# Symb0x76/ChineseChessZero

Measured on AMD Instinct MI355X. Metric: self-play MCTS simulations/sec, higher is better.
Workload: dtype u8 rules / f32 Q (reference CPU path) / f64 PUCT (net: fp16)

## Files before the change

chinesechesszero_amd/_lib.py:

```python
from __future__ import annotations

import ctypes as C
import os

import torch

_HERE = os.path.dirname(os.path.abspath(__file__))
LIB_PATH = os.path.join(_HERE, "libcczero.so")

NSQ = 90
SQ_STRIDE = 96
NMOVES = 2086
MAX_LEGAL = 128
MASK_WORDS = 66
PLANES = 10710
REC_BYTES, REC_HDR, REC_IDS, REC_PI = 880, 96, 112, 368
HEAD_POL_STRIDE, HEAD_VAL_STRIDE = 1536, 640

ABI_VERSION = 8
CONV_RELU, CONV_DESCENDING, CONV_FORCE_SMALL, CONV_FORCE_TILE, CONV_G16, CONV_G16_EDGE_TILES = 1, 2, 16, 32, 64, 128
CONV_G16_ONE_LAUNCH = 512
RULE_PERPETUAL_CHECK = 1
RULE_PAWN_MOVE_RESETS_CLOCK = 2
FLAG_REFERENCE_QUIRKS = 1
# ... 46 lines not shown
    "ccz_last_error": (C.c_char_p, []),
    "ccz_device_count": (C.c_int, []),
    "ccz_action_table": (C.c_int, [_P, _P, _P]),
    "ccz_flip_map": (C.c_int, [_P]),
    "ccz_create": (C.c_int, [C.POINTER(Config), C.POINTER(_P)]),
    "ccz_destroy": (C.c_int, [_P]),
    "ccz_reset": (C.c_int, [_P, _P, _P]),
    "ccz_set_position": (C.c_int, [_P, _P, C.c_int32, _P, C.c_int32, C.c_int32]),
    "ccz_reset_tree": (C.c_int, [_P, _P, _P]),
    "ccz_select_leaves": (C.c_int, [_P, _P, _P]),
    "ccz_zero_leaf_input": (C.c_int, [_P, _P, _P]),
    "ccz_expand_backup": (C.c_int, [_P, _P, _P, _P]),
    "ccz_step": (C.c_int, [_P, _P, _P, _P, _P]),
    "ccz_gather_priors": (C.c_int, [_P, _P, _P, C.c_int32]),
    "ccz_step_compact": (C.c_int, [_P, _P, _P, _P]),
    "ccz_expand_backup_compact": (C.c_int, [_P, _P, _P]),
    "ccz_eval_plan": (C.c_int, [_P, _P, _P, _P]),
    "ccz_set_scouts": (C.c_int, [_P, C.c_int32]),
    "ccz_scout": (C.c_int, [_P, _P, _P]),
    "ccz_eval_plan_scouted": (C.c_int, [_P, _P, _P, _P, _P]),
    "ccz_scout_and_plan": (C.c_int, [_P, _P, _P, _P, _P, _P]),
    "ccz_scouted_run": (C.c_int, [_P, _P, _P, _P, _P, _P, _P]),
    "ccz_gather_priors_planned": (C.c_int, [_P, _P, _P, C.c_int32, _P]),
    "ccz_eval_cache_clear": (C.c_int, [_P, _P]),
    "ccz_set_routing": (C.c_int, [_P, _P, _P, C.c_uint64, C.c_uint64]),
    "ccz_eval_plan_routed": (C.c_int, [_P, _P, _P, _P]),
    "ccz_gather_priors_routed": (C.c_int, [_P, _P, _P, _P, C.c_int32, _P, _P]),
    "ccz_finish_move": (C.c_int, [_P, _P, _P, _P, _P, C.c_int32]),
    "ccz_root_children": (C.c_int, [_P, _P, _P, _P, _P, _P, _P, _P]),
    "ccz_root_pi": (C.c_int, [_P, _P, _P, _P]),
    "ccz_move_distribution": (C.c_int, [_P, _P, _P, _P, _P, _P]),
    "ccz_game_status": (C.c_int, [_P, _P, _P, _P, _P, _P]),
    "ccz_root_positions": (C.c_int, [_P, _P, _P]),
    "ccz_leaf_info": (C.c_int, [_P, _P, _P, _P, _P, _P]),
    "ccz_leaf_priors": (C.c_int, [_P, _P, _P, _P]),
    "ccz_leaf_keys": (C.c_int, [_P, _P, _P, _P]),
    "ccz_harvest_rows": (C.c_int, [_P, _P, C.POINTER(C.c_int64)]),
    "ccz_harvest": (C.c_int, [_P, _P, _P, _P, _P, C.c_int64, C.POINTER(C.c_int64)]),
    "ccz_harvest_records": (C.c_int, [_P, _P, _P, C.c_int64, C.POINTER(C.c_int64)]),
    "ccz_expand_records": (C.c_int, [_P, _P, C.c_int64, C.c_uint32, _P, _P, _P, _P, C.c_int64, C.c_int64, _P]),
    "ccz_ring_retire": (C.c_int, [_P, _P, C.c_int64, _P, C.c_int64, C.c_int32, _P]),
    "ccz_sample_records": (C.c_int, [_P, _P, C.c_int64, _P, _P, C.c_int64, C.c_uint32, _P, _P, _P, _P, _P]),
    "ccz_get_stats": (C.c_int, [_P, _P, C.POINTER(Stats)]),
    "ccz_legal_moves": (C.c_int, [_P, C.c_int32, _P, _P, _P, _P, _P, _P]),
    "ccz_apply_moves": (C.c_int, [_P, C.c_int32, _P, _P, _P, _P]),
    "ccz_bias_act_f16": (C.c_int, [_P, _P, _P, _P, C.c_int64, C.c_int32]),
# ... 73 lines not shown
```

chinesechesszero_amd/csrc/cczero.hip:

```cpp
#include "../../include/cczero.h"

#include <hip/hip_runtime.h>

#include <cmath>
#include <cstdarg>
#include <cstdio>
#include <cstring>
#include <new>
#include <vector>

#include "cczero_kernels.h"
#include "cczero_netops.h"
#include "cczero_conv.h"
#include "cczero_conv_small.h"
#include "cczero_conv_g16.h"
#include "cczero_conv_g16e.h"
#include "cczero_heads.h"

using namespace ccz;

namespace {

thread_local char g_err[512] = "";

// ... 504 lines not shown
    return 0;
}

int ccz_eval_cache_clear(ccz_engine *e, void *stream)
{
    NEED(e);
    if (!e->d.cache) return 0;
    hipStream_t s = (hipStream_t)stream;
    HIP_TRY(hipMemsetAsync(e->d.cache, 0, ((size_t)e->d.cache_mask + 1) * sizeof(CacheEntry), s));
    HIP_TRY(hipMemsetAsync(e->d.claim, 0x7f, ((size_t)e->d.cache_mask + 1) * 4, s));
    return 0;
}

int ccz_step_compact(ccz_engine *e, void *stream, const float *value_dev, void *leaf_input_f16_dev)
{
    NEED(e);
    if (!value_dev && !e->d.cache) return fail(-1, "ccz_step_compact: null value (engine-owned leaf values exist only with an evaluation cache)");
    hipLaunchKernelGGL(k_step<true>, dim3(ACTIVE(e)), dim3(64), 0, (hipStream_t)stream, e->d, (const float *)e->d.prior128, value_dev,
                       (uint16_t *)leaf_input_f16_dev);
    HIP_TRY(hipGetLastError());
    return 0;
}

int ccz_expand_backup_compact(ccz_engine *e, void *stream, const float *value_dev)
{
    NEED(e);
    if (!value_dev && !e->d.cache) return fail(-1, "ccz_expand_backup_compact: null value (engine-owned leaf values exist only with an evaluation cache)");
    hipLaunchKernelGGL(k_expand_backup<true>, dim3(ACTIVE(e)), dim3(64), 0, (hipStream_t)stream, e->d, (const float *)e->d.prior128,
                       value_dev);
    HIP_TRY(hipGetLastError());
    return 0;
}

int ccz_finish_move(ccz_engine *e, void *stream, const int32_t *forced_moves_dev, const double *temps_dev,
                    int32_t *moves_out_dev, int32_t keep_tree)
{
    NEED(e);
    hipLaunchKernelGGL(k_finish_move, dim3(ACTIVE(e)), dim3(64), 0, (hipStream_t)stream, e->d, forced_moves_dev, temps_dev,
                       moves_out_dev, keep_tree ? 1 : 0);
    HIP_TRY(hipGetLastError());
    hipLaunchKernelGGL(k_flip_half, dim3(1), dim3(1), 0, (hipStream_t)stream, e->d);
    HIP_TRY(hipGetLastError());
    return 0;
}

int ccz_root_children(ccz_engine *e, void *stream, int32_t *k_host, uint16_t *acts_host, int32_t *visits_host,
// ... 663 lines not shown
```

chinesechesszero_amd/csrc/cczero_kernels.h:

```cpp
#pragma once
#include "cczero_device.h"

namespace ccz {

constexpr uint16_t kHalfOne = 0x3C00;
constexpr int kMaxDepth = 512;

__device__ __forceinline__ void set_err(const Dev &D, int bit) { atomicOr(D.err, bit); }

__device__ __forceinline__ int start_piece(int s)
{
    const int r = s / 9, f = s - 9 * r;
    const int rr = r <= 4 ? r : 9 - r;
    const int add = r <= 4 ? 0 : 8;
    int t = 0;
    if (rr == 0) {
        const int ff = f <= 4 ? f : 8 - f;
        t = ff == 0 ? ROOK : ff == 1 ? KNIGHT : ff == 2 ? BISHOP : ff == 3 ? ADVISOR : KING;
    } else if (rr == 2) {
        t = (f == 1 || f == 7) ? CANNON : 0;
    } else if (rr == 3) {
        t = (f & 1) ? 0 : PAWN;
    }
    return t ? t + add : 0;
// ... 399 lines not shown
        if (lane == 0) { D.leaf_status[b] = CCZ_LEAF_NONE; D.leaf_k[b] = 0; D.path_len[b] = 0; }
        return;
    }
    if (lane < 24) {
        uint32_t v = P.sqw;
        if (lane == 22) v &= 0x0000ffffu;
        if (lane == 23) v = 0u;
        ((uint32_t *)sh.sq)[lane] = v;
    }
    sh.chain[lane] = P.c0;
    if (P.m.chain_len > 64) sh.chain[64 + lane] = D.chain[(size_t)r * kChainCap + 64 + lane];
    if (lane >= 1 && lane < d) sh.pm.mv[lane - 1] = (uint16_t)(Bn[CCZ_IDX(D, pj, D.cap)] & 0xffffu);
    if (lane == 0) sh.pm.mv[d - 1] = (uint16_t)(Bn[CCZ_IDX(D, sib, D.cap)] & 0xffffu);
    wave_sync();
    leaf_tail(D, b, lane, leaf_in, sh, d, P.m.turn, P.m.halfmove, P.m.chain_len, P.m.key, false);
}

__global__ __launch_bounds__(64) void k_scout(Dev D, uint16_t *leaf_in, int active)
{
    __shared__ SelectShared sh;
    scout_wave(D, leaf_in, active, blockIdx.x, threadIdx.x, sh);
}

template <bool COMPACT>
__device__ inline TopPatch expand_backup_phase(const Dev &D, int b, int lane, const float *prob, const float *value,
                                               const BoardMeta &m0, int half)
{
    TopPatch tp;
    tp.active = false; tp.root_expanded = false; tp.kid_expanded = false; tp.k = 0; tp.first_id = 0; tp.n0 = 0; tp.rootN = 0;
    tp.rootQ = 0.0f; tp.node1 = -1; tp.N1 = 0; tp.Q1 = 0.0f; tp.has1 = false;
    const int status = D.leaf_status[b];
    const int d = D.path_len[b];
    const int k_leaf = D.leaf_k[b];
    const float v_net = value ? value[b] : D.vleaf[b];
    const int32_t *path = D.path + (size_t)b * D.maxd;
    const uint16_t *ids = D.leaf_ids + (size_t)b * kMaxLegal;
    const int id0 = ids[lane], id1 = ids[64 + lane];
    float cp0 = 0.0f, cp1 = 0.0f;
    if (COMPACT) { cp0 = prob[(size_t)b * kMaxLegal + lane]; cp1 = prob[(size_t)b * kMaxLegal + 64 + lane]; }
    const int pj = path[lane < D.maxd ? lane : 0];
    if (status == CCZ_LEAF_SKIP) return tp;
    CCZ_STAMP(D, b, lane, 8)
    BoardMeta *mp = D.meta + b;
    const size_t base = ((size_t)b * 2 + half) * (size_t)D.cap;
    NodeA *A = D.nodeA + base;
    uint32_t *Bn = D.nodeB + base;
    const int leaf = __builtin_amdgcn_readlane(pj, __builtin_amdgcn_readfirstlane(d < 64 ? d : 0));
    float v;
    if (status == CCZ_LEAF_EXPAND) {
        const int k = k_leaf;
        const int n0 = m0.n_nodes;
        v = v_net;
        if (n0 + k > D.cap) {
            set_err(D, 1);
        } else {
            const float *pr = prob + (size_t)b * kNMoves;
            if (lane < k) {
                A[CCZ_IDX(D, n0 + lane, D.cap)] = NodeA{0, 0.0f, COMPACT ? cp0 : pr[COMPACT ? 0 : CCZ_IDX(D, id0, kNMoves)], -1};
                Bn[CCZ_IDX(D, n0 + lane, D.cap)] = (uint32_t)id0;
            }
            if (64 + lane < k) {
                A[CCZ_IDX(D, n0 + 64 + lane, D.cap)] = NodeA{0, 0.0f, COMPACT ? cp1 : pr[COMPACT ? 0 : CCZ_IDX(D, id1, kNMoves)], -1};
// ... 69 lines not shown
    __shared__ SelectShared sh;
    const int b = blockIdx.x, lane = threadIdx.x;
    CCZ_STAMP(D, b, lane, 0)
    const Prefetch P = prefetch_board(D, b, lane);
    const TopPatch tp = expand_backup_phase<COMPACT>(D, b, lane, prob, value, P.m, P.half);
    CCZ_STAMP(D, b, lane, 1)
    __threadfence_block();
    __syncthreads();
    CCZ_STAMP(D, b, lane, 2)
    select_phase(D, b, lane, leaf_in, sh, P, tp);
    CCZ_STAMP(D, b, lane, 9)
}

__device__ __forceinline__ uint32_t cache_tag(int id0, int id1, int k, int lane)
{
    uint64_t h = 0;
    if (lane < k) h ^= mix64(((uint64_t)(uint32_t)id0 << 8 | (uint32_t)lane) + 0x9E3779B97F4A7C15ull);
    if (64 + lane < k) h ^= mix64(((uint64_t)(uint32_t)id1 << 8 | (uint32_t)(64 + lane)) + 0x9E3779B97F4A7C15ull);
    h = wave_readlane64(wave_incl_xor64(h), 63);
    return ((uint32_t)(h >> 40) << 8) | (uint32_t)(k & 0xff);
}

template <typename T, bool PLANNED>
__device__ __forceinline__ void softmax_gather_board(const Dev &D, int b, int lane, float *row, const T *logits, const float *vcompact,
                                                     uint64_t salt)
{
    const int status = D.leaf_status[b];
    int cst = 0, src = b;
    if (PLANNED) {
        cst = D.cstate[b];
        src = D.row_of[b];
    }
    const int k = D.leaf_k[b];
    const uint16_t *ids = D.leaf_ids + (size_t)b * kMaxLegal;
    const int id0 = ids[lane], id1 = ids[64 + lane];
    if (status != CCZ_LEAF_EXPAND || cst != 0) return;
    const T *srcrow = logits + (size_t)src * kNMoves;
    float mx = -__builtin_huge_valf();
    float sum = 0.0f;
    if constexpr (sizeof(T) == 2) {
        static_assert(kNMoves % 2 == 0, "dword rows");
        const uint32_t *src32 = (const uint32_t *)srcrow;
        constexpr int kIt = (kNMoves / 2 + 63) / 64;
        uint32_t wreg[kIt];
#pragma unroll
        for (int i = 0; i < kIt; ++i) {
            const int j = lane + 64 * i;
            wreg[i] = j < kNMoves / 2 ? src32[j] : 0u;
        }
#pragma unroll
        for (int i = 0; i < kIt; ++i) {
            const int j = lane + 64 * i;
            if (j < kNMoves / 2) {
                const uint32_t w = wreg[i];
                const float x0 = (float)__builtin_bit_cast(_Float16, (uint16_t)(w & 0xffffu));
                const float x1 = (float)__builtin_bit_cast(_Float16, (uint16_t)(w >> 16));
                *(float2 *)(row + 2 * j) = make_float2(x0, x1);
                mx = fmaxf(mx, fmaxf(x0, x1));
            }
// ... 24 lines not shown
            const bool d0 = lane < k && __float_as_uint(out[lane]) != __float_as_uint(p0);
            const bool d1 = 64 + lane < k && __float_as_uint(out[64 + lane]) != __float_as_uint(p1);
            const bool dv = __float_as_uint(D.vleaf[b]) != __float_as_uint(v);
            const bool bad = __ballot(d0 || d1 || dv) != 0ull;
            if (lane == 0) {
                D.stats[b].cache_verified += 1u;
                if (bad) D.stats[b].cache_mismatch += 1u;
            }
        }
        if (lane < k) out[lane] = p0;
        if (64 + lane < k) out[64 + lane] = p1;
        const uint32_t slot = D.cslot[b];
        if (lane == 0) {
            D.vleaf[b] = v;
            D.claim[slot] = 0x7fffffff;
        }
        if (D.cins[b]) {
            CacheEntry *e = D.cache + slot;
            const uint32_t tag = cache_tag(id0, id1, k, lane);
            e->pri[lane] = p0;
            e->pri[64 + lane] = p1;
            if (lane == 0) { e->v = v; e->k = tag; e->key = D.leaf_key[b] ^ salt; D.stats[b].cache_stores += 1u; }
        }
    } else {
        if (lane < k) out[lane] = p0;
        if (64 + lane < k) out[64 + lane] = p1;
    }
}

template <typename T, bool PLANNED>
__global__ __launch_bounds__(64) void k_softmax_gather(Dev D, const T *logits, const float *vcompact)
{
    __shared__ __attribute__((aligned(16))) float row[kNMoves + 2];
    softmax_gather_board<T, PLANNED>(D, blockIdx.x, threadIdx.x, row, logits, vcompact, 0ull);
}

template <typename T>
__global__ __launch_bounds__(64) void k_softmax_gather_routed(Dev D, const uint8_t *net, const T *logits0, const T *logits1,
                                                              const float *v0, const float *v1, uint64_t salt0, uint64_t salt1)
{
    __shared__ __attribute__((aligned(16))) float row[kNMoves + 2];
    const int b = blockIdx.x;
    const int n = net[b];
    softmax_gather_board<T, true>(D, b, threadIdx.x, row, n ? logits1 : logits0, n ? v1 : v0, n ? salt1 : salt0);
}

__device__ __forceinline__ uint32_t cache_slot(uint64_t key, uint32_t mask) { return (uint32_t)(key ^ (key >> 29)) & mask; }

__device__ inline int cache_probe_wave(const Dev &D, int b, int lane, uint64_t salt = 0)
{
    const int status = D.leaf_status[b];
    const uint64_t key = D.leaf_key[b] ^ salt;
    if (status != CCZ_LEAF_EXPAND) {
        if (lane == 0) D.cstate[b] = 2;
        return 2;
    }
    const uint32_t slot = cache_slot(key, D.cache_mask);
// ... 887 lines not shown
```

chinesechesszero_amd/engine.py:

```python
from __future__ import annotations

import ctypes as C

import numpy as np
import torch

from . import _lib
from ._lib import MAX_LEGAL, NMOVES, SQ_STRIDE, CczError, Config, Stats, check


def _ptr(t):
    if t is None:
        return None
    if isinstance(t, torch.Tensor):
        return C.c_void_p(t.data_ptr())
    if isinstance(t, np.ndarray):
        return C.c_void_p(t.ctypes.data)
    raise TypeError(type(t))


class SelfPlayEngine:
    def __init__(self, n_boards: int, n_playout: int = 400, c_puct: float = 5, eps: float = 0.25,
                 alpha: float = 0.2, temp: float = 1.0, seed: int = 0, board_id_base: int = 0,
                 device: int = 0, max_nodes: int = 0, max_depth: int = 0, max_plies: int = 0,
# ... 31 lines not shown
            cfg.move_rank_host = self.move_rank.ctypes.data
        self.plane_of_type = (0, 0, 1, 2, 3, 4, 5, 6) if plane_of_type is None else tuple(int(x) for x in plane_of_type)
        if plane_of_type is not None:
            cfg.plane_of_type = (C.c_uint8 * 8)(*self.plane_of_type)
        if isinstance(pawn_move_resets_clock, str):
            pawn_move_resets_clock = tools.PAWN_MOVE_RESETS_CLOCK
        self.pawn_move_resets_clock = bool(pawn_move_resets_clock)
        if isinstance(perpetual_check, str):
            perpetual_check = tools.PERPETUAL_CHECK
        self.perpetual_check = bool(perpetual_check)
        cfg.rule_flags = (_lib.RULE_PAWN_MOVE_RESETS_CLOCK if self.pawn_move_resets_clock else 0) \
            | (_lib.RULE_PERPETUAL_CHECK if self.perpetual_check else 0)
        self.type_rank = None if type_rank is None else tuple(int(x) for x in type_rank)
        if self.type_rank is not None:
            if len(self.type_rank) != 8:
                raise ValueError("type_rank must have 8 entries")
            cfg.type_rank = (C.c_uint8 * 8)(*self.type_rank)
        self.eval_cache_log2 = int(eval_cache_log2)
        cfg.eval_cache_log2 = self.eval_cache_log2
        h = C.c_void_p()
        with torch.cuda.device(self.device):
            check(self.L.ccz_create(C.byref(cfg), C.byref(h)))
        self.h = h
        self.miss_rows = torch.zeros((self.B,), dtype=torch.int32, device=self.device)
        self.n_miss = torch.zeros((1,), dtype=torch.int32, device=self.device)
        self.leaf_input = torch.zeros((self.B, 17, 7, 10, 9), dtype=torch.float16, device=self.device)
        self.moves_out = torch.full((self.B,), -1, dtype=torch.int32, device=self.device)
        self._forced = torch.full((self.B,), -1, dtype=torch.int32, device=self.device)
        self._temps = torch.ones((self.B,), dtype=torch.float64, device=self.device)

    def close(self):
        if getattr(self, "h", None) is not None and self.h.value:
            self.L.ccz_destroy(self.h)
            self.h = C.c_void_p()

    def __del__(self):
        try:
            self.close()
        except Exception:
            pass

    def _stream(self):
        return C.c_void_p(torch.cuda.current_stream(self.device).cuda_stream)

    def reset(self, mask=None):
        m = None if mask is None else np.ascontiguousarray(mask, dtype=np.uint8)
        check(self.L.ccz_reset(self.h, self._stream(), _ptr(m)))

    def reset_tree(self, mask=None):
        m = None if mask is None else np.ascontiguousarray(mask, dtype=np.uint8)
        check(self.L.ccz_reset_tree(self.h, self._stream(), _ptr(m)))

    def set_position(self, board: int, squares, turn: int, halfmove: int = 0):
        sq = np.ascontiguousarray(squares, dtype=np.uint8)
        assert sq.shape == (90,)
        check(self.L.ccz_set_position(self.h, self._stream(), int(board), _ptr(sq), int(turn), int(halfmove)))

    def select_leaves(self) -> torch.Tensor:
        check(self.L.ccz_select_leaves(self.h, self._stream(), _ptr(self.leaf_input)))
        return self.leaf_input

    def expand_backup(self, prob: torch.Tensor, value: torch.Tensor):
        if prob.dtype != torch.float32 or value.dtype != torch.float32:
            raise TypeError("prob and value must be float32")
        if tuple(prob.shape) != (self.B, NMOVES) or value.numel() != self.B:
# ... 17 lines not shown
            raise TypeError("logits must be float16/float32 and value float32")
        if tuple(logits.shape) != (self.B, NMOVES) or value.numel() != self.B:
            raise ValueError(f"logits must be [{self.B},{NMOVES}] and value [{self.B}]")
        if not (logits.is_cuda and value.is_cuda and logits.is_contiguous() and value.is_contiguous()):
            raise ValueError("logits/value must be contiguous device tensors")
        return 1 if logits.dtype == torch.float16 else 0

    def step_logits(self, logits: torch.Tensor, value: torch.Tensor) -> torch.Tensor:
        self.gather_priors(logits, value)
        return self.step_compact(value)

    def expand_backup_logits(self, logits: torch.Tensor, value: torch.Tensor):
        self.gather_priors(logits, value)
        check(self.L.ccz_expand_backup_compact(self.h, self._stream(), _ptr(value)))

    def gather_priors(self, logits: torch.Tensor, value: torch.Tensor):
        f16 = self._check_logits(logits, value)
        check(self.L.ccz_gather_priors(self.h, self._stream(), _ptr(logits), f16))

    def expand_backup_compact(self, value: torch.Tensor | None):
        check(self.L.ccz_expand_backup_compact(self.h, self._stream(), _ptr(value)))

    def step_compact(self, value: torch.Tensor | None) -> torch.Tensor:
        check(self.L.ccz_step_compact(self.h, self._stream(), _ptr(value), _ptr(self.leaf_input)))
        return self.leaf_input

    def eval_plan(self):
        check(self.L.ccz_eval_plan(self.h, self._stream(), _ptr(self.miss_rows), _ptr(self.n_miss)))
        return self.miss_rows, self.n_miss

    def set_scouts(self, n_scouts: int):
        check(self.L.ccz_set_scouts(self.h, int(n_scouts)))
        self.n_scouts = int(n_scouts)
        if not hasattr(self, "_plan_state_host"):
            self._plan_state_host = torch.zeros((self.B,), dtype=torch.int32).pin_memory()

    def scout(self):
        check(self.L.ccz_scout(self.h, self._stream(), _ptr(self.leaf_input)))

    def plan_scouted_launch(self):
        check(self.L.ccz_eval_plan_scouted(self.h, self._stream(), _ptr(self.miss_rows), _ptr(self.n_miss),
                                           C.c_void_p(self._plan_state_host.data_ptr())))

    def scout_and_plan(self):
        check(self.L.ccz_scout_and_plan(self.h, self._stream(), _ptr(self.leaf_input), _ptr(self.miss_rows), _ptr(self.n_miss),
                                        C.c_void_p(self._plan_state_host.data_ptr())))
# ... 7 lines not shown
    def set_run(self, budget: int, left: int):
        if budget < 1 or left < 1:
            raise ValueError("scouted run: budget and simulations left must be >= 1")
        if not hasattr(self, "_run_host"):
            self._run_host = torch.zeros((4,), dtype=torch.int32).pin_memory()
            self._run_np = self._run_host.numpy()
        self._run_np[0] = budget
        self._run_np[1] = left

    def run_outcome(self):
        torch.cuda.current_stream(self.device).synchronize()
        return int(self._run_np[2]), bool(self._run_np[3])

    def plan_state_of_board0(self) -> int:
        torch.cuda.current_stream(self.device).synchronize()
        return int(self._plan_state_host[0])

    def plan_states(self) -> np.ndarray:
        torch.cuda.current_stream(self.device).synchronize()
        return self._plan_state_host[: self.B - self.n_scouts].numpy().copy()

    def gather_priors_planned(self, logits: torch.Tensor, value: torch.Tensor):
        f16 = self._check_logits(logits, value)
        check(self.L.ccz_gather_priors_planned(self.h, self._stream(), _ptr(logits), f16, _ptr(value)))

    def step_planned(self, logits: torch.Tensor, value: torch.Tensor) -> torch.Tensor:
        self.gather_priors_planned(logits, value)
        return self.step_compact(None)

    def expand_backup_planned(self, logits: torch.Tensor, value: torch.Tensor):
        self.gather_priors_planned(logits, value)
        check(self.L.ccz_expand_backup_compact(self.h, self._stream(), None))

    def clear_eval_cache(self):
        check(self.L.ccz_eval_cache_clear(self.h, self._stream()))

    def set_routing(self, red_net, salts=(0, 0)):
        if red_net is None:
            check(self.L.ccz_set_routing(self.h, self._stream(), None, 0, 0))
            return
        rn = np.ascontiguousarray(red_net, dtype=np.uint8)
        if rn.shape != (self.B,):
            raise ValueError(f"red_net must have {self.B} entries")
        s0, s1 = (int(x) & (2**64 - 1) for x in salts)
        with torch.cuda.device(self.device):
            check(self.L.ccz_set_routing(self.h, self._stream(), _ptr(rn), s0, s1))
        if not hasattr(self, "miss_rows2"):
# ... 249 lines not shown
```

chinesechesszero_amd/net.py:

```python
from __future__ import annotations

import os

import numpy as np
import torch
import torch.nn.functional as F
from torch import nn

PIECES = 7
PLAYS = 17


class ResBlock(nn.Module):

    def __init__(self, num_channels=256):
        super().__init__()
        self.conv1 = nn.Conv2d(num_channels, num_channels, kernel_size=(3, 3), stride=(1, 1), padding=1)
        self.conv1_bn = nn.BatchNorm2d(num_channels)
        self.conv1_act = nn.ReLU()
        self.conv2 = nn.Conv2d(num_channels, num_channels, kernel_size=(3, 3), stride=(1, 1), padding=1)
        self.conv2_bn = nn.BatchNorm2d(num_channels)
        self.conv2_act = nn.ReLU()

    def forward(self, x):
# ... 33 lines not shown
        value = self.value_act2(self.value_fc1(torch.reshape(value, [-1, PIECES * 10 * 9])))
        value = torch.tanh(self.value_fc2(value))
        return policy, value


def _fold(conv: nn.Conv2d, bn: nn.BatchNorm2d):
    scale = bn.weight.detach().double() / torch.sqrt(bn.running_var.detach().double() + bn.eps)
    w = conv.weight.detach().double() * scale.view(-1, 1, 1, 1)
    b = (conv.bias.detach().double() - bn.running_mean.detach().double()) * scale + bn.bias.detach().double()
    return w, b


def pack_conv_weights_g16(w):
    co, cin = w.shape[0], w.shape[-1]
    w5 = w.reshape(co, 9, cin // 32, 4, 8)
    f = (-(torch.arange(co, device=w.device) >> 2)) & 3
    idx = torch.arange(4, device=w.device)[None, :] ^ f[:, None]
    w5 = torch.gather(w5, 3, idx[:, None, None, :, None].expand(co, 9, cin // 32, 4, 8))
    return w5.permute(2, 1, 0, 3, 4).contiguous().view(cin // 32, 9, co, 32)


class EvalOptions:

    FIELDS = ("fused_conv", "fused_stem", "fused_heads", "fused_last", "layout", "force", "groups", "chains", "zigzag", "edge_tiles", "one_launch")

    def __init__(self, env=None):
        env = os.environ if env is None else env
        self.fused_conv = env.get("CCZ_FUSED_CONV", "1") != "0"
        self.fused_stem = env.get("CCZ_FUSED_STEM", "1") != "0"
        self.fused_heads = env.get("CCZ_FUSED_HEADS", "1") != "0"
        self.fused_last = env.get("CCZ_FUSED_LAST", "1") != "0"
        self.layout = env.get("CCZ_CONV_LAYOUT", "auto")
        self.force = {"small": 16, "tile": 32}.get(env.get("CCZ_CONV_FORCE", ""), 0)
        self.groups = int(env.get("CCZ_TOWER_GROUPS", "0"))
        self.chains = int(env.get("CCZ_TOWER_CHAINS", "0"))
        self.zigzag = env.get("CCZ_CONV_ZIGZAG", "1") == "1"
        self.edge_tiles = {"0": False, "1": True}.get(env.get("CCZ_CONV_EDGE_TILES", "auto"), "auto")
        self.one_launch = env.get("CCZ_CONV_ONE_LAUNCH", "1") != "0"
        if self.layout not in ("auto", "nhwc", "g16"):
            raise ValueError("CCZ_CONV_LAYOUT must be auto, nhwc or g16")

    def non_default(self):
        d = EvalOptions(env={})
        return {f: getattr(self, f) for f in self.FIELDS if getattr(self, f) != getattr(d, f)}


_CHAIN_STREAMS: dict = {}
CHAIN_STREAM_PRIORITY = -1
N_CHAIN_STREAMS = 8


def chain_streams(device):
    device = torch.device(device)
    if device.index is None:
        device = torch.device("cuda", torch.cuda.current_device())
    got = _CHAIN_STREAMS.get(device)
    if got is None:
        got = [torch.cuda.Stream(device=device, priority=CHAIN_STREAM_PRIORITY) for _ in range(N_CHAIN_STREAMS)]
        cur = torch.cuda.current_stream(device)
        ev = torch.cuda.Event()
        ev.record(cur)
# ... 155 lines not shown
            y = y + residual
        return F.relu_(y)

    FUSED_MIN_BOARDS = 1

    def _use_fused_tower(self, x) -> bool:
        if not self.opt.fused_conv:
            return False
        return bool(x.is_cuda and x.dtype == torch.float16 and x.shape[1] == 256 and x.shape[0] >= self.FUSED_MIN_BOARDS
                    and x.is_contiguous(memory_format=torch.channels_last))

    G16_MIN_BOARDS = 640

    def _g16(self, B) -> bool:
        mode = self.opt.layout
        if mode == "nhwc" or self.opt.force:
            return False
        return B >= (65 if mode == "g16" else self.G16_MIN_BOARDS)

    TOWER_GROUP_BOARDS_G16 = 4096
    TOWER_GROUP_BOARDS = 2048
    TOWER_CHAINS = 2

    def _tower_fused(self, x, plan=None, g16=None, heads=None):
        import ctypes as C
        from . import _lib
        L = _lib.lib()
        if g16 is None:
            g16 = self._g16(x.shape[0]) and x.shape[0] % 16 == 0
        y = torch.empty_like(x)
        Bt = x.shape[0]
        groups = self.tower_groups(Bt, g16)
        if torch.cuda.is_current_stream_capturing():
            groups = 1
        if plan is not None:
            self._tower_planned(L, C, x, y, plan, groups, g16, heads)
            return x
        gstep = -(-(-(-Bt // groups)) // 128) * 128 if groups > 1 else Bt
        for g0 in range(0, Bt, gstep):
            self._tower_range(L, C, x, y, g0, min(Bt, g0 + gstep), g16, heads)
        return x

    def _tower_planned(self, L, C, x, y, plan, groups, g16=False, heads=None):
        from . import _lib
        B = x.shape[0]
        cur = torch.cuda.current_stream(x.device)
        edge = self._edge(B, g16)
        chains = 1 if torch.cuda.is_current_stream_capturing() else self.tower_chains(B, groups, edge)
        n_parts = groups * chains
        if g16:
            cap = -(-(B // 16) // n_parts) * 1440
        else:
            cap = -(-(-(-B // n_parts)) // 8) * 8 * 90
        lay = (_lib.CONV_G16 | self._edge_flags(edge)) if g16 else 0
        pool = self._chain_pool(x.device, chains) if chains > 1 else None
        live = C.c_void_p(plan[1].data_ptr())
        xp, yp = C.c_void_p(x.data_ptr()), C.c_void_p(y.data_ptr())
        down = 2 if self.opt.zigzag else 0
        for g in range(groups):
            streams = [cur] if chains == 1 else pool[:chains]
            if chains > 1:
                fork = torch.cuda.Event()
                fork.record(cur)
                for st in streams:
                    st.wait_event(fork)
            wsrc = self.ws_g16 if g16 else self.ws
            for i in range(0, len(self.ws), 2):
                w1, b1_, w2, b2_ = (C.c_void_p(t.data_ptr()) for t in (wsrc[i], self.bs32[i], wsrc[i + 1], self.bs32[i + 1]))
                for k, st in enumerate(streams):
                    _lib.check(L.ccz_conv3x3_c256_f16_live(C.c_void_p(st.cuda_stream), xp, w1, b1_, None, yp, cap, 1 | down | lay, live, g * chains + k, n_parts))
                if heads is not None and i == len(self.ws) - 2:
                    hw, hb, hp, hv = (C.c_void_p(t.data_ptr()) for t in (self.head_w32, self.head_b32, heads[0], heads[1]))
                    for k, st in enumerate(streams):
                        _lib.check(L.ccz_conv3x3_c256_heads_f16(C.c_void_p(st.cuda_stream), yp, w2, b2_, xp, hw, hb, hp, hv, cap, 1 | lay, live, g * chains + k, n_parts))
                    continue
                for k, st in enumerate(streams):
                    _lib.check(L.ccz_conv3x3_c256_f16_live(C.c_void_p(st.cuda_stream), yp, w2, b2_, xp, xp, cap, 1 | lay, live, g * chains + k, n_parts))
            for st in (streams if chains > 1 else []):
                join = torch.cuda.Event()
                join.record(st)
                cur.wait_event(join)

    def _tower_range(self, L, C, x, y, lo, hi, g16=False, heads=None):
        from . import _lib
        B = hi - lo
        cur = torch.cuda.current_stream(x.device)
        edge = self._edge(x.shape[0], g16)
        parts = 1 if torch.cuda.is_current_stream_capturing() else self.tower_chains(B, 1, edge)
        step = -(-B // parts)
# ... 26 lines not shown
                    _lib.check(L.ccz_conv3x3_c256_heads_f16(s, yp, w2, b2_, xp, hw, hb, hp, hv, n_pixels, 1 | v2, None, 0, 1))
                continue
            for _, s, xp, yp, n_pixels, _b0 in chains:
                _lib.check(L.ccz_conv3x3_c256_f16(s, yp, w2, b2_, xp, xp, n_pixels, 1 | v2))
        for st, *_ in (chains if len(chains) > 1 else []):
            join = torch.cuda.Event()
            join.record(st)
            cur.wait_event(join)

    def _chain_pool(self, device, n):
        pool = getattr(self, "_chain_streams", None)
        if pool is None or pool[0] != device or len(pool[1]) < n:
            pool = (device, chain_streams(device))
            self._chain_streams = pool
        return pool[1]

    def _edge_flags(self, edge: bool) -> int:
        from . import _lib
        return (_lib.CONV_G16_EDGE_TILES | (_lib.CONV_G16_ONE_LAUNCH if self.opt.one_launch else 0)) if edge else 0

    def _force_flag(self) -> int:
        return self.opt.force

    def _stem_fused(self, leaf_input, plan=None, g16=None):
        import ctypes as C
        from . import _lib
        L = _lib.lib()
        B = leaf_input.shape[0]
        if g16 is None:
            g16 = self._g16(B)
        s = C.c_void_p(torch.cuda.current_stream(leaf_input.device).cuda_stream)
        Bp = -(-B // 16) * 16 if g16 else B
        lay = _lib.CONV_G16 if g16 else 0
        if plan is None:
            x64 = (torch.zeros if Bp != B else torch.empty)((Bp, 90, 64), dtype=torch.float16, device=leaf_input.device)
            y = torch.empty((Bp, 256, 10, 9), dtype=torch.float16, device=leaf_input.device, memory_format=torch.channels_last)
            if g16:
                _lib.check(L.ccz_pack_live_planes_g16_f16(s, C.c_void_p(leaf_input.data_ptr()), C.c_void_p(x64.data_ptr()), B, None, None))
            else:
                _lib.check(L.ccz_pack_live_planes_f16(s, C.c_void_p(leaf_input.data_ptr()), C.c_void_p(x64.data_ptr()), B))
            _lib.check(L.ccz_conv3x3_stem_f16(s, C.c_void_p(x64.data_ptr()), C.c_void_p((self.stem_w64_g16 if g16 else self.stem_w64).data_ptr()), C.c_void_p(self.stem_b32.data_ptr()),
                                              C.c_void_p(y.data_ptr()), Bp * 90, 1 | self._force_flag() | lay))
            return y
        rows, n_rows = plan
        bufs = self.__dict__.setdefault("_plan_bufs", {})
        key = (Bp, leaf_input.device, g16)
        if key not in bufs:
            bufs[key] = (torch.zeros((Bp, 90, 64), dtype=torch.float16, device=leaf_input.device),
                         torch.empty((Bp, 256, 10, 9), dtype=torch.float16, device=leaf_input.device, memory_format=torch.channels_last).zero_())
        x64, y = bufs[key]
        pack = L.ccz_pack_live_planes_g16_f16 if g16 else L.ccz_pack_live_planes_rows_f16
        _lib.check(pack(s, C.c_void_p(leaf_input.data_ptr()), C.c_void_p(x64.data_ptr()), B, C.c_void_p(rows.data_ptr()), C.c_void_p(n_rows.data_ptr())))
        _lib.check(L.ccz_conv3x3_stem_f16_live(s, C.c_void_p(x64.data_ptr()), C.c_void_p((self.stem_w64_g16 if g16 else self.stem_w64).data_ptr()), C.c_void_p(self.stem_b32.data_ptr()),
                                               C.c_void_p(y.data_ptr()), Bp * 90 if g16 else -(-B // 8) * 8 * 90, 1 | lay, C.c_void_p(n_rows.data_ptr()), 0, 1))
        return y

    @torch.no_grad()
    def tower_activations(self, leaf_input):
        B = leaf_input.shape[0]
        g16 = self._g16(B)
        x = self._tower_fused(self._stem_fused(leaf_input, None, g16), None, g16)
        if not g16:
            return x
        Bp, Cn = x.shape[0], x.shape[1]
        rows = x.permute(0, 2, 3, 1).reshape(Bp // 16, 90, 16, Cn).permute(0, 2, 1, 3).reshape(Bp, 10, 9, Cn)[:B]
        return rows.permute(0, 3, 1, 2)

    def _path(self, leaf_input) -> str:
        B = leaf_input.shape[0]
        key = (B, leaf_input.is_cuda, leaf_input.dtype, leaf_input.is_contiguous())
        cache = self.__dict__.setdefault("_path_cache", {})
        if key not in cache:
            o = self.opt
            fused = (hasattr(self, "stem_w64") and leaf_input.is_cuda and leaf_input.dtype == torch.float16 and leaf_input.is_contiguous()
                     and B >= self.FUSED_MIN_BOARDS and self.dtype == torch.float16 and o.fused_conv and o.fused_stem)
            if fused:
                cache[key] = "g16" if self._g16(B) else "nhwc"
            else:
                cache[key] = "torch_stem" if (o.fused_conv and leaf_input.is_cuda and self.dtype == torch.float16
                                              and self.ws and self.ws[0].shape[0] == 256 and self.ws[0].shape[1] == 256) else "torch"
        return cache[key]

    @torch.no_grad()
    def forward(self, leaf_input: torch.Tensor, return_logits: bool = False, plan=None):
        B = leaf_input.shape[0]
        path = self._path(leaf_input)
        if plan is not None and path not in ("g16", "nhwc"):
            leaf_input = leaf_input.index_select(0, plan[0].long().clamp_(0, B - 1))
            plan = None
        g16 = path == "g16"
        if path in ("g16", "nhwc"):
            x = self._stem_fused(leaf_input, plan, g16)
            probe = self.__dict__.get("tower_probe")
            if probe is not None:
                p0, p1 = torch.cuda.Event(enable_timing=True), torch.cuda.Event(enable_timing=True)
                p0.record()
            heads = self._head_buffers(x.shape[0], x.device)[:2] if (g16 and self.opt.fused_last and self._fused_heads_ok(x)) else None
            x = self._tower_fused(x, plan, g16, heads)
            if probe is not None:
                p1.record()
                probe.append((p0, p1))
            if heads is not None:
                return self._heads(x, B, g16, plan, return_logits, conv_done=True)
        else:
            x = leaf_input.view(B, PLAYS * PIECES, 10, 9)
            if self.live_only:
                x = torch.cat([x[:, 49:56], x[:, 105:119]], dim=1)
            x = x.to(self.dtype).contiguous(memory_format=torch.channels_last)
            x = self._epilogue(F.conv2d(x, self.stem_w, None, padding=1), self.stem_b)
            if path == "torch_stem" and self._use_fused_tower(x):
                x = self._tower_fused(x, None, False)
            else:
                if x.is_cuda and x.dtype == torch.float16 and self.opt.fused_conv:
                    key = (int(x.shape[0]), int(x.shape[1]))
                    seen = self.__dict__.setdefault("_off_fused_seen", set())
                    if key not in seen:
                        seen.add(key)
                        from .tools import log
                        log(f"evaluator: batch of {key[0]} boards x {key[1]} channels is off the fused tower kernels "
                            f"(k_conv3x3_g16 / k_conv3x3_small serve 256-channel towers): MIOpen convolutions + one-pass epilogue")
                for i in range(0, len(self.ws), 2):
# ... 197 lines not shown
```

chinesechesszero_amd/selfplay.py:

```python
from __future__ import annotations

import os

import numpy as np
import torch

from .engine import SelfPlayEngine
from .parameters import ALPHA, C_PUCT, EPS


class GraphedStep:

    def __init__(self, engine: SelfPlayEngine, evaluator, warmup: int = 3, version_fn=None):
        self.engine = engine
        self.evaluator = evaluator
        self.warmup = warmup
        self.captures = 0
        self.version_fn = version_fn
        if version_fn is None and not hasattr(getattr(evaluator, "__self__", None), "weights_version") \
                and not getattr(evaluator, "stateless", False) and getattr(evaluator, "__name__", "") != "uniform_evaluator":
            from .tools import log
            log("GraphedStep: the evaluator exposes no weights_version and no version_fn was given: the captured hipGraph will "
                "keep replaying the weights it was captured with (pass version_fn=... if they can change)", "WARNING")
        self._capture()
# ... 150 lines not shown
    def __init__(self, evaluator, n_boards: int, n_playout: int = 400, c_puct: float = C_PUCT, eps: float = EPS,
                 alpha: float = ALPHA, temp: float = 1.0, seed: int = 0, board_id_base: int = 0, device: int = 0,
                 sampling: str = "device", use_graph: bool = False, version_fn=None, **engine_kw):
        if sampling not in ("device", "numpy"):
            raise ValueError("sampling must be 'device' (Philox on the GPU) or 'numpy' (reference-exact host RNG)")
        self.evaluator = evaluator
        self.engine = SelfPlayEngine(n_boards, n_playout=n_playout, c_puct=c_puct, eps=eps, alpha=alpha, temp=temp,
                                     seed=seed, board_id_base=board_id_base, device=device, **engine_kw)
        self.B = n_boards
        self.n_playout = n_playout
        self.sampling = sampling
        self.eps, self.alpha, self.temp = eps, alpha, temp
        self.rngs = [np.random.RandomState((seed + board_id_base + b) % (2**32)) for b in range(n_boards)] if sampling == "numpy" else None
        self.use_graph = use_graph
        self._graph = None
        self.planned = bool(self.engine.eval_cache_log2 > 0 and getattr(evaluator, "accepts_plan", False)
                            and getattr(evaluator, "returns_logits", False))
        self.version_fn = version_fn
        if self.planned and version_fn is None and not hasattr(getattr(evaluator, "__self__", None), "weights_version") \
                and not getattr(evaluator, "stateless", False):
            raise ValueError("planned evaluator boundary (evaluation cache) with an evaluator that exposes no weights_version: "
                             "pass version_fn=... (what changes when its weights do), mark it `stateless = True`, or use eval_cache_log2=0")
        self._cache_version = self._evaluator_version()
        self._sim = 0
        self._leaf = None
        self._acc = 0

    def _evaluator_version(self):
        if self.version_fn is not None:
            return self.version_fn()
        return getattr(getattr(self.evaluator, "__self__", None), "weights_version", None)

    def _planned_eval(self, leaf):
        e = self.engine
        v = self._evaluator_version()
        if v != self._cache_version:
            e.clear_eval_cache()
            self._cache_version = v
        return self.evaluator(leaf, plan=e.eval_plan())

    def simulate(self):
        e = self.engine
        leaf = e.select_leaves()
        if self.planned:
            e.expand_backup_planned(*self._planned_eval(leaf))
            return
        prob, value = self.evaluator(leaf)
        (e.expand_backup_logits if getattr(self.evaluator, "returns_logits", False) else e.expand_backup)(prob, value)

# ... 109 lines not shown
```

include/cczero.h:

```cpp
#ifndef CCZERO_H
#define CCZERO_H

#include <stdint.h>

#ifdef __cplusplus
extern "C" {
#endif

#define CCZ_ABI_VERSION 8
#define CCZ_NSQ 90
#define CCZ_SQ_STRIDE 96
#define CCZ_NMOVES 2086
#define CCZ_MAX_LEGAL 128
#define CCZ_MASK_WORDS 66
#define CCZ_PLANES 10710


#define CCZ_RULE_PAWN_MOVE_RESETS_CLOCK 2u
#define CCZ_RULE_PERPETUAL_CHECK 1u

#define CCZ_FLAG_REFERENCE_QUIRKS 1u
#define CCZ_FLAG_NO_MIRROR 2u
#define CCZ_FLAG_VALUE_F16 4u

// ... 81 lines not shown

int ccz_select_leaves(ccz_engine *e, void *stream, void *leaf_input_f16_dev);
int ccz_zero_leaf_input(ccz_engine *e, void *stream, void *leaf_input_f16_dev);
int ccz_expand_backup(ccz_engine *e, void *stream, const float *prob_dev, const float *value_dev);

int ccz_step(ccz_engine *e, void *stream, const float *prob_dev, const float *value_dev,
             void *leaf_input_f16_dev);

int ccz_gather_priors(ccz_engine *e, void *stream, const void *logits_dev, int32_t logits_f16);
int ccz_step_compact(ccz_engine *e, void *stream, const float *value_dev, void *leaf_input_f16_dev);
int ccz_expand_backup_compact(ccz_engine *e, void *stream, const float *value_dev);

int ccz_set_scouts(ccz_engine *e, int32_t n_scouts);
int ccz_scout(ccz_engine *e, void *stream, void *leaf_input_f16_dev);
int ccz_eval_plan_scouted(ccz_engine *e, void *stream, int32_t *miss_rows_dev, int32_t *n_miss_dev, int32_t *state_dev);
int ccz_scout_and_plan(ccz_engine *e, void *stream, void *leaf_input_f16_dev, int32_t *miss_rows_dev, int32_t *n_miss_dev, int32_t *state_dev);
int ccz_scouted_run(ccz_engine *e, void *stream, void *leaf_input_f16_dev, int32_t *miss_rows_dev, int32_t *n_miss_dev, int32_t *state_dev,
                    int32_t *run_dev);

int ccz_eval_plan(ccz_engine *e, void *stream, int32_t *miss_rows_dev, int32_t *n_miss_dev);
int ccz_gather_priors_planned(ccz_engine *e, void *stream, const void *logits_compact_dev, int32_t logits_f16,
                              const float *value_compact_dev);
int ccz_eval_cache_clear(ccz_engine *e, void *stream);

int ccz_set_routing(ccz_engine *e, void *stream, const uint8_t *red_net_host, uint64_t salt0, uint64_t salt1);
int ccz_eval_plan_routed(ccz_engine *e, void *stream, int32_t *miss_rows_dev, int32_t *n_miss_dev);
int ccz_gather_priors_routed(ccz_engine *e, void *stream, const void *logits0_dev, const void *logits1_dev, int32_t logits_f16,
                             const float *value0_dev, const float *value1_dev);

int ccz_finish_move(ccz_engine *e, void *stream, const int32_t *forced_moves_dev,
                    const double *temps_dev, int32_t *moves_out_dev, int32_t keep_tree);

int ccz_root_children(ccz_engine *e, void *stream, int32_t *k_host, uint16_t *acts_host,
                      int32_t *visits_host, float *q_host, float *prior_host, int32_t *root_visits_host);
int ccz_root_pi(ccz_engine *e, void *stream, const double *temps_host, double *pi_host);
int ccz_move_distribution(ccz_engine *e, void *stream, const double *temps_host, double *gamma_host, double *mixed_host,
                          double *u_host);
int ccz_game_status(ccz_engine *e, void *stream, uint8_t *over_host, int8_t *winner_host,
                    int32_t *plies_host, uint8_t *turn_host);
int ccz_root_positions(ccz_engine *e, void *stream, uint8_t *sq_host);
int ccz_leaf_info(ccz_engine *e, void *stream, uint8_t *status_host, int32_t *k_host,
                  uint16_t *ids_host, int32_t *depth_host);

int ccz_leaf_priors(ccz_engine *e, void *stream, float *prior_host, float *value_host);

int ccz_leaf_keys(ccz_engine *e, void *stream, uint64_t *keys_dev, uint8_t *status_dev);
// ... 76 lines not shown
```

Before: 193,000.

## Fuse planned prior gather into MCTS step kernel and run stem per tower chain

Adds a k_step_planned kernel that performs the softmax/prior gather and the expand-backup-select step in one launch. Freshly computed priors and value are passed in registers instead of being written to and reread from the cache or prior buffer. The Python side defers the gather call so the next step_compact can use the fused path, and flushes any pending gather before other stream use. Separately, the network stem conv is moved into the per-chain tower streams instead of running as one launch before the fork. The gain is fewer launches and less global memory traffic, at the cost of more state-dependent deferred-call logic and a larger shared-memory union in the fused kernel.

```diff
diff --git a/chinesechesszero_amd/_lib.py b/chinesechesszero_amd/_lib.py
--- a/chinesechesszero_amd/_lib.py
+++ b/chinesechesszero_amd/_lib.py
@@ -92,6 +92,7 @@
     "ccz_scout_and_plan": (C.c_int, [_P, _P, _P, _P, _P, _P]),
     "ccz_scouted_run": (C.c_int, [_P, _P, _P, _P, _P, _P, _P]),
     "ccz_gather_priors_planned": (C.c_int, [_P, _P, _P, C.c_int32, _P]),
+    "ccz_step_planned": (C.c_int, [_P, _P, _P, C.c_int32, _P, _P]),
     "ccz_eval_cache_clear": (C.c_int, [_P, _P]),
     "ccz_set_routing": (C.c_int, [_P, _P, _P, C.c_uint64, C.c_uint64]),
     "ccz_eval_plan_routed": (C.c_int, [_P, _P, _P, _P]),
diff --git a/chinesechesszero_amd/csrc/cczero.hip b/chinesechesszero_amd/csrc/cczero.hip
--- a/chinesechesszero_amd/csrc/cczero.hip
+++ b/chinesechesszero_amd/csrc/cczero.hip
@@ -550,6 +550,24 @@
     return 0;
 }
 
+int ccz_step_planned(ccz_engine *e, void *stream, const void *logits_compact_dev, int32_t logits_f16, const float *value_compact_dev,
+                     void *leaf_input_f16_dev)
+{
+    NEED(e);
+    if (!e->d.cache) return fail(-1, "ccz_step_planned: the engine was created without an evaluation cache");
+    if (e->active > 0) return fail(-1, "ccz_step_planned: not with scout slots (ccz_set_scouts): the gather runs on every slot, the step on the searched boards");
+    if (!logits_compact_dev || !value_compact_dev) return fail(-1, "ccz_step_planned: null logits / value");
+    hipStream_t s = (hipStream_t)stream;
+    if (logits_f16)
+        hipLaunchKernelGGL(k_step_planned<_Float16>, dim3(e->d.B), dim3(64), 0, s, e->d, (const _Float16 *)logits_compact_dev, value_compact_dev,
+                           (uint16_t *)leaf_input_f16_dev);
+    else
+        hipLaunchKernelGGL(k_step_planned<float>, dim3(e->d.B), dim3(64), 0, s, e->d, (const float *)logits_compact_dev, value_compact_dev,
+                           (uint16_t *)leaf_input_f16_dev);
+    HIP_TRY(hipGetLastError());
+    return 0;
+}
+
 int ccz_expand_backup_compact(ccz_engine *e, void *stream, const float *value_dev)
 {
     NEED(e);
diff --git a/chinesechesszero_amd/csrc/cczero_kernels.h b/chinesechesszero_amd/csrc/cczero_kernels.h
--- a/chinesechesszero_amd/csrc/cczero_kernels.h
+++ b/chinesechesszero_amd/csrc/cczero_kernels.h
@@ -445,9 +445,14 @@
     scout_wave(D, leaf_in, active, blockIdx.x, threadIdx.x, sh);
 }
 
+struct FreshEval {
+    bool have;
+    float p0, p1, v;
+};
+
 template <bool COMPACT>
 __device__ inline TopPatch expand_backup_phase(const Dev &D, int b, int lane, const float *prob, const float *value,
-                                               const BoardMeta &m0, int half)
+                                               const BoardMeta &m0, int half, const FreshEval fe = FreshEval{false, 0.0f, 0.0f, 0.0f})
 {
     TopPatch tp;
     tp.active = false; tp.root_expanded = false; tp.kid_expanded = false; tp.k = 0; tp.first_id = 0; tp.n0 = 0; tp.rootN = 0;
@@ -455,12 +460,15 @@
     const int status = D.leaf_status[b];
     const int d = D.path_len[b];
     const int k_leaf = D.leaf_k[b];
-    const float v_net = value ? value[b] : D.vleaf[b];
+    const float v_net = fe.have ? fe.v : (value ? value[b] : D.vleaf[b]);
     const int32_t *path = D.path + (size_t)b * D.maxd;
     const uint16_t *ids = D.leaf_ids + (size_t)b * kMaxLegal;
     const int id0 = ids[lane], id1 = ids[64 + lane];
     float cp0 = 0.0f, cp1 = 0.0f;
-    if (COMPACT) { cp0 = prob[(size_t)b * kMaxLegal + lane]; cp1 = prob[(size_t)b * kMaxLegal + 64 + lane]; }
+    if (COMPACT) {
+        if (fe.have) { cp0 = fe.p0; cp1 = fe.p1; }
+        else { cp0 = prob[(size_t)b * kMaxLegal + lane]; cp1 = prob[(size_t)b * kMaxLegal + 64 + lane]; }
+    }
     const int pj = path[lane < D.maxd ? lane : 0];
     if (status == CCZ_LEAF_SKIP) return tp;
     CCZ_STAMP(D, b, lane, 8)
@@ -576,8 +584,8 @@
 }
 
 template <typename T, bool PLANNED>
-__device__ __forceinline__ void softmax_gather_board(const Dev &D, int b, int lane, float *row, const T *logits, const float *vcompact,
-                                                     uint64_t salt)
+__device__ __forceinline__ FreshEval softmax_gather_board(const Dev &D, int b, int lane, float *row, const T *logits, const float *vcompact,
+                                                          uint64_t salt)
 {
     const int status = D.leaf_status[b];
     int cst = 0, src = b;
@@ -588,7 +596,7 @@
     const int k = D.leaf_k[b];
     const uint16_t *ids = D.leaf_ids + (size_t)b * kMaxLegal;
     const int id0 = ids[lane], id1 = ids[64 + lane];
-    if (status != CCZ_LEAF_EXPAND || cst != 0) return;
+    if (status != CCZ_LEAF_EXPAND || cst != 0) return FreshEval{false, 0.0f, 0.0f, 0.0f};
     const T *srcrow = logits + (size_t)src * kNMoves;
     float mx = -__builtin_huge_valf();
     float sum = 0.0f;
@@ -659,17 +667,40 @@
             e->pri[64 + lane] = p1;
             if (lane == 0) { e->v = v; e->k = tag; e->key = D.leaf_key[b] ^ salt; D.stats[b].cache_stores += 1u; }
         }
+        return FreshEval{true, p0, p1, v};
     } else {
         if (lane < k) out[lane] = p0;
         if (64 + lane < k) out[64 + lane] = p1;
     }
+    return FreshEval{false, 0.0f, 0.0f, 0.0f};
 }
 
 template <typename T, bool PLANNED>
 __global__ __launch_bounds__(64) void k_softmax_gather(Dev D, const T *logits, const float *vcompact)
 {
     __shared__ __attribute__((aligned(16))) float row[kNMoves + 2];
-    softmax_gather_board<T, PLANNED>(D, blockIdx.x, threadIdx.x, row, logits, vcompact, 0ull);
+    (void)softmax_gather_board<T, PLANNED>(D, blockIdx.x, threadIdx.x, row, logits, vcompact, 0ull);
+}
+
+template <typename T>
+__global__ __launch_bounds__(64) void k_step_planned(Dev D, const T *logits, const float *vcompact, uint16_t *leaf_in)
+{
+    union StepPlannedShared {
+        __attribute__((aligned(16))) float row[kNMoves + 2];
+        SelectShared sh;
+    };
+    __shared__ StepPlannedShared u;
+    const int b = blockIdx.x, lane = threadIdx.x;
+    CCZ_STAMP(D, b, lane, 0)
+    const Prefetch P = prefetch_board(D, b, lane);
+    const FreshEval fe = softmax_gather_board<T, true>(D, b, lane, u.row, logits, vcompact, 0ull);
+    const TopPatch tp = expand_backup_phase<true>(D, b, lane, D.prior128, nullptr, P.m, P.half, fe);
+    CCZ_STAMP(D, b, lane, 1)
+    __threadfence_block();
+    __syncthreads();
+    CCZ_STAMP(D, b, lane, 2)
+    select_phase(D, b, lane, leaf_in, u.sh, P, tp);
+    CCZ_STAMP(D, b, lane, 9)
 }
 
 template <typename T>
diff --git a/chinesechesszero_amd/engine.py b/chinesechesszero_amd/engine.py
--- a/chinesechesszero_amd/engine.py
+++ b/chinesechesszero_amd/engine.py
@@ -77,6 +77,9 @@
         with torch.cuda.device(self.device):
             check(self.L.ccz_create(C.byref(cfg), C.byref(h)))
         self.h = h
+        self.fuse_planned_step = False
+        self._pending_gather = None
+        self.n_scouts = getattr(self, "n_scouts", 0)
         self.miss_rows = torch.zeros((self.B,), dtype=torch.int32, device=self.device)
         self.n_miss = torch.zeros((1,), dtype=torch.int32, device=self.device)
         self.leaf_input = torch.zeros((self.B, 17, 7, 10, 9), dtype=torch.float16, device=self.device)
@@ -85,6 +88,7 @@
         self._temps = torch.ones((self.B,), dtype=torch.float64, device=self.device)
 
     def close(self):
+        self._pending_gather = None
         if getattr(self, "h", None) is not None and self.h.value:
             self.L.ccz_destroy(self.h)
             self.h = C.c_void_p()
@@ -96,6 +100,10 @@
             pass
 
     def _stream(self):
+        if self._pending_gather is not None:
+            logits, value, f16 = self._pending_gather
+            self._pending_gather = None
+            check(self.L.ccz_gather_priors_planned(self.h, self._stream(), _ptr(logits), f16, _ptr(value)))
         return C.c_void_p(torch.cuda.current_stream(self.device).cuda_stream)
 
     def reset(self, mask=None):
@@ -159,6 +167,11 @@
         check(self.L.ccz_expand_backup_compact(self.h, self._stream(), _ptr(value)))
 
     def step_compact(self, value: torch.Tensor | None) -> torch.Tensor:
+        if value is None and self._pending_gather is not None:
+            logits, v, f16 = self._pending_gather
+            self._pending_gather = None
+            check(self.L.ccz_step_planned(self.h, self._stream(), _ptr(logits), f16, _ptr(v), _ptr(self.leaf_input)))
+            return self.leaf_input
         check(self.L.ccz_step_compact(self.h, self._stream(), _ptr(value), _ptr(self.leaf_input)))
         return self.leaf_input
 
@@ -212,7 +225,11 @@
 
     def gather_priors_planned(self, logits: torch.Tensor, value: torch.Tensor):
         f16 = self._check_logits(logits, value)
-        check(self.L.ccz_gather_priors_planned(self.h, self._stream(), _ptr(logits), f16, _ptr(value)))
+        stream = self._stream()
+        if self.fuse_planned_step and not self.n_scouts and self.eval_cache_log2 > 0:
+            self._pending_gather = (logits, value, f16)
+            return
+        check(self.L.ccz_gather_priors_planned(self.h, stream, _ptr(logits), f16, _ptr(value)))
 
     def step_planned(self, logits: torch.Tensor, value: torch.Tensor) -> torch.Tensor:
         self.gather_priors_planned(logits, value)
diff --git a/chinesechesszero_amd/net.py b/chinesechesszero_amd/net.py
--- a/chinesechesszero_amd/net.py
+++ b/chinesechesszero_amd/net.py
@@ -79,7 +79,8 @@
 
 class EvalOptions:
 
-    FIELDS = ("fused_conv", "fused_stem", "fused_heads", "fused_last", "layout", "force", "groups", "chains", "zigzag", "edge_tiles", "one_launch")
+    FIELDS = ("fused_conv", "fused_stem", "fused_heads", "fused_last", "layout", "force", "groups", "chains", "zigzag", "edge_tiles", "one_launch",
+              "stem_per_chain")
 
     def __init__(self, env=None):
         env = os.environ if env is None else env
@@ -94,6 +95,7 @@
         self.zigzag = env.get("CCZ_CONV_ZIGZAG", "1") == "1"
         self.edge_tiles = {"0": False, "1": True}.get(env.get("CCZ_CONV_EDGE_TILES", "auto"), "auto")
         self.one_launch = env.get("CCZ_CONV_ONE_LAUNCH", "1") != "0"
+        self.stem_per_chain = env.get("CCZ_STEM_PER_CHAIN", "1") != "0"
         if self.layout not in ("auto", "nhwc", "g16"):
             raise ValueError("CCZ_CONV_LAYOUT must be auto, nhwc or g16")
 
@@ -295,7 +297,7 @@
     TOWER_GROUP_BOARDS = 2048
     TOWER_CHAINS = 2
 
-    def _tower_fused(self, x, plan=None, g16=None, heads=None):
+    def _tower_fused(self, x, plan=None, g16=None, heads=None, stem=None):
         import ctypes as C
         from . import _lib
         L = _lib.lib()
@@ -307,14 +309,14 @@
         if torch.cuda.is_current_stream_capturing():
             groups = 1
         if plan is not None:
-            self._tower_planned(L, C, x, y, plan, groups, g16, heads)
+            self._tower_planned(L, C, x, y, plan, groups, g16, heads, stem)
             return x
         gstep = -(-(-(-Bt // groups)) // 128) * 128 if groups > 1 else Bt
         for g0 in range(0, Bt, gstep):
             self._tower_range(L, C, x, y, g0, min(Bt, g0 + gstep), g16, heads)
         return x
 
-    def _tower_planned(self, L, C, x, y, plan, groups, g16=False, heads=None):
+    def _tower_planned(self, L, C, x, y, plan, groups, g16=False, heads=None, stem=None):
         from . import _lib
         B = x.shape[0]
         cur = torch.cuda.current_stream(x.device)
@@ -338,6 +340,11 @@
                 for st in streams:
                     st.wait_event(fork)
             wsrc = self.ws_g16 if g16 else self.ws
+            if stem is not None:
+                sw, sb, sx = (C.c_void_p(t.data_ptr()) for t in (self.stem_w64_g16 if g16 else self.stem_w64, self.stem_b32, stem))
+                for k, st in enumerate(streams):
+                    _lib.check(L.ccz_conv3x3_stem_f16_live(C.c_void_p(st.cuda_stream), sx, sw, sb, xp, cap, 1 | (_lib.CONV_G16 if g16 else 0), live,
+                                                           g * chains + k, n_parts))
             for i in range(0, len(self.ws), 2):
                 w1, b1_, w2, b2_ = (C.c_void_p(t.data_ptr()) for t in (wsrc[i], self.bs32[i], wsrc[i + 1], self.bs32[i + 1]))
                 for k, st in enumerate(streams):
@@ -410,7 +417,7 @@
     def _force_flag(self) -> int:
         return self.opt.force
 
-    def _stem_fused(self, leaf_input, plan=None, g16=None):
+    def _stem_fused(self, leaf_input, plan=None, g16=None, pack_only=False):
         import ctypes as C
         from . import _lib
         L = _lib.lib()
@@ -439,6 +446,8 @@
         x64, y = bufs[key]
         pack = L.ccz_pack_live_planes_g16_f16 if g16 else L.ccz_pack_live_planes_rows_f16
         _lib.check(pack(s, C.c_void_p(leaf_input.data_ptr()), C.c_void_p(x64.data_ptr()), B, C.c_void_p(rows.data_ptr()), C.c_void_p(n_rows.data_ptr())))
+        if pack_only:
+            return x64, y
         _lib.check(L.ccz_conv3x3_stem_f16_live(s, C.c_void_p(x64.data_ptr()), C.c_void_p((self.stem_w64_g16 if g16 else self.stem_w64).data_ptr()), C.c_void_p(self.stem_b32.data_ptr()),
                                                C.c_void_p(y.data_ptr()), Bp * 90 if g16 else -(-B // 8) * 8 * 90, 1 | lay, C.c_void_p(n_rows.data_ptr()), 0, 1))
         return y
@@ -478,13 +487,17 @@
             plan = None
         g16 = path == "g16"
         if path in ("g16", "nhwc"):
-            x = self._stem_fused(leaf_input, plan, g16)
+            stem = None
+            if plan is not None and self.opt.stem_per_chain:
+                stem, x = self._stem_fused(leaf_input, plan, g16, pack_only=True)
+            else:
+                x = self._stem_fused(leaf_input, plan, g16)
             probe = self.__dict__.get("tower_probe")
             if probe is not None:
                 p0, p1 = torch.cuda.Event(enable_timing=True), torch.cuda.Event(enable_timing=True)
                 p0.record()
             heads = self._head_buffers(x.shape[0], x.device)[:2] if (g16 and self.opt.fused_last and self._fused_heads_ok(x)) else None
-            x = self._tower_fused(x, plan, g16, heads)
+            x = self._tower_fused(x, plan, g16, heads, stem)
             if probe is not None:
                 p1.record()
                 probe.append((p0, p1))
diff --git a/chinesechesszero_amd/selfplay.py b/chinesechesszero_amd/selfplay.py
--- a/chinesechesszero_amd/selfplay.py
+++ b/chinesechesszero_amd/selfplay.py
@@ -196,9 +196,18 @@
             raise ValueError("planned evaluator boundary (evaluation cache) with an evaluator that exposes no weights_version: "
                              "pass version_fn=... (what changes when its weights do), mark it `stateless = True`, or use eval_cache_log2=0")
         self._cache_version = self._evaluator_version()
+        self.fuse_step = self.planned and os.environ.get("CCZ_STEP_FUSED", "1") != "0"
         self._sim = 0
         self._leaf = None
         self._acc = 0
+
+    @property
+    def fuse_step(self) -> bool:
+        return bool(getattr(self.engine, "fuse_planned_step", False))
+
+    @fuse_step.setter
+    def fuse_step(self, on):
+        self.engine.fuse_planned_step = bool(on)
 
     def _evaluator_version(self):
         if self.version_fn is not None:
diff --git a/include/cczero.h b/include/cczero.h
--- a/include/cczero.h
+++ b/include/cczero.h
@@ -127,6 +127,8 @@
 int ccz_gather_priors_planned(ccz_engine *e, void *stream, const void *logits_compact_dev, int32_t logits_f16,
                               const float *value_compact_dev);
 int ccz_eval_cache_clear(ccz_engine *e, void *stream);
+int ccz_step_planned(ccz_engine *e, void *stream, const void *logits_compact_dev, int32_t logits_f16, const float *value_compact_dev,
+                     void *leaf_input_f16_dev);
 
 int ccz_set_routing(ccz_engine *e, void *stream, const uint8_t *red_net_host, uint64_t salt0, uint64_t salt1);
 int ccz_eval_plan_routed(ccz_engine *e, void *stream, int32_t *miss_rows_dev, int32_t *n_miss_dev);
```

After: 193,300, median of 4. Within noise of the previous version (+0.2%).
